# YifanXu74/MQ-Det

Hardware: AMD Instinct MI355X
Metric: images/sec MQ-GLIP-T 800×1333 5-shot vision queries, 1/2/4/8 MI355X (higher is better)
Workload: dtype f16; 1 GPU; BASELINE.json configs[1]: MQ-GLIP-T (Swin-T + BERT-base + GCP + 6-layer VLDyHead), 5 vision queries x 40 classes, 141-token caption, LVIS-style post-processing; every step a full forward (feature / language caches OFF; only host-side tokenizer / query-selection results are memoised)); global_batch=8, batch_per_gpu=8, image=800x1333 -> 800x1344, parallelism=dp1, weights=seeded random init (no checkpoints offline), residual_streams=fp32

## Files before the change

mq_det_amd/csrc/common.h:

```cpp
#pragma once
#include <hip/hip_runtime.h>
#include <stdint.h>

#if defined(MQ_F32)
typedef float half_t;
typedef float half8 __attribute__((ext_vector_type(8)));
typedef float half4 __attribute__((ext_vector_type(4)));
typedef float half2_ __attribute__((ext_vector_type(2)));
#define MQ_SYM(name) name##_f32
#define MQ_NAMESPACE_BEGIN namespace mq_f32 {
#define MQ_NAMESPACE_END }
#elif defined(MQ_BF16)
typedef __bf16 half_t;
typedef __bf16 half8 __attribute__((ext_vector_type(8)));
typedef __bf16 half4 __attribute__((ext_vector_type(4)));
typedef __bf16 half2_ __attribute__((ext_vector_type(2)));
#define MQ_SYM(name) name##_bf16
#define MQ_NAMESPACE_BEGIN namespace mq_bf16 {
#define MQ_NAMESPACE_END }
#else
typedef _Float16 half_t;
typedef _Float16 half8 __attribute__((ext_vector_type(8)));
typedef _Float16 half4 __attribute__((ext_vector_type(4)));
typedef _Float16 half2_ __attribute__((ext_vector_type(2)));
#define MQ_SYM(name) name
#define MQ_NAMESPACE_BEGIN
#define MQ_NAMESPACE_END
#endif
#if !defined(MQ_BF16) && !defined(MQ_F32)
#define MQ_PRIMARY_UNIT 1
#endif
#if defined(MQ_F32)
#define __expf(x) expf(x)
#define __builtin_amdgcn_exp2f(x) exp2f(x)
#define __builtin_amdgcn_rcpf(x) (1.0f / (x))
#endif
typedef float float4_ __attribute__((ext_vector_type(4)));
typedef float float2_ __attribute__((ext_vector_type(2)));

#define MQ_NEG_BIG (-1.0e30f)

#if defined(MQ_F32) && !defined(MQ_F32_EXACT)
typedef _Float16 mq_h16x8 __attribute__((ext_vector_type(8)));
struct mq_split8 { mq_h16x8 hi, lo; };
__device__ __forceinline__ mq_split8 mq_split(half8 x) {
  mq_split8 s;
#pragma unroll
  for (int i = 0; i < 8; ++i) {
    const _Float16 h = (_Float16)x[i];
    s.hi[i] = h;
    s.lo[i] = (_Float16)(__builtin_fmaf((float)h, -1.0f, x[i]) * 2048.0f);
  }
  return s;
}
__device__ __forceinline__ float4_ mfma16_split(const mq_split8& a, const mq_split8& b, float4_ c) {
#if defined(MQ_SIMT_EMULATION)
  return simt_mfma_16x16x32_split_frag(a.hi, a.lo, b.hi, b.lo, c);
#else
  float4_ t = {0.f, 0.f, 0.f, 0.f};
  c = __builtin_amdgcn_mfma_f32_16x16x32_f16(a.hi, b.hi, c, 0, 0, 0);
  t = __builtin_amdgcn_mfma_f32_16x16x32_f16(a.hi, b.lo, t, 0, 0, 0);
  t = __builtin_amdgcn_mfma_f32_16x16x32_f16(a.lo, b.hi, t, 0, 0, 0);
#pragma unroll
  for (int r = 0; r < 4; ++r) c[r] = __builtin_fmaf(t[r], 1.0f / 2048.0f, c[r]);
  return c;
#endif
}
typedef _Float16 mq_h16x4 __attribute__((ext_vector_type(4)));
typedef float mq_f32x4 __attribute__((ext_vector_type(4)));
__device__ __forceinline__ void mq_split4(mq_f32x4 x, mq_h16x4& hi, mq_h16x4& lo) {
#pragma unroll
  for (int i = 0; i < 4; ++i) {
    const _Float16 h = (_Float16)x[i];
    hi[i] = h;
    lo[i] = (_Float16)(__builtin_fmaf((float)h, -1.0f, x[i]) * 2048.0f);
  }
}
#endif

__device__ __forceinline__ float4_ mfma16(half8 a, half8 b, float4_ c) {
#if defined(MQ_F32) && !defined(MQ_F32_EXACT)
#if defined(MQ_SIMT_EMULATION)
  return simt_mfma_16x16x32_split(a, b, c);
#else
  return mfma16_split(mq_split(a), mq_split(b), c);
#endif
#elif defined(MQ_F32)
#if defined(MQ_SIMT_EMULATION)
  return simt_mfma_16x16x32_f32_8x4(a, b, c);
#else
#pragma unroll
  for (int j = 0; j < 8; ++j) c = __builtin_amdgcn_mfma_f32_16x16x4f32(a[j], b[j], c, 0, 0, 0);
  return c;
#endif
#elif defined(MQ_BF16)
  return __builtin_amdgcn_mfma_f32_16x16x32_bf16(a, b, c, 0, 0, 0);
#else
  return __builtin_amdgcn_mfma_f32_16x16x32_f16(a, b, c, 0, 0, 0);
#endif
}

__device__ __forceinline__ half8 zero8() {
  half8 z;
#pragma unroll
  for (int i = 0; i < 8; ++i) z[i] = (half_t)0.f;
  return z;
}

typedef __fp16 mq_fp16x4_t __attribute__((__vector_size__(8)));
__device__ __forceinline__ half4 lds_read_tr16(const half_t* p) {
#if defined(MQ_F32)
  const int l = __lane_id(), base = l & ~15, i = l & 15;
  half4 o;
#pragma unroll
  for (int j = 0; j < 4; ++j) {
    const half_t* src = (const half_t*)__shfl((unsigned long long)p, base + 4 * j + (i >> 2));
    o[j] = src[i & 3];
  }
  return o;
#else
  mq_fp16x4_t v = __builtin_amdgcn_ds_read_tr16_b64_v4f16((__attribute__((address_space(3))) mq_fp16x4_t*)p);
  half4 o;
  __builtin_memcpy(&o, &v, 8);
  return o;
#endif
}

typedef _Float16 mq_h16x4_t __attribute__((ext_vector_type(4)));
__device__ __forceinline__ mq_h16x4_t lds_read_tr16_h(const _Float16* p) {
  mq_fp16x4_t v = __builtin_amdgcn_ds_read_tr16_b64_v4f16((__attribute__((address_space(3))) mq_fp16x4_t*)p);
  mq_h16x4_t o;
  __builtin_memcpy(&o, &v, 8);
  return o;
}

__device__ __forceinline__ void lds_stage_frag8(const half_t* src_lane, half_t* dst_base, int lane) {
#if defined(MQ_F32)
  *(half8*)(dst_base + lane * 8) = *(const half8*)src_lane;
  asm volatile("s_waitcnt lgkmcnt(0)" ::: "memory");
#else
  (void)lane;
  __builtin_amdgcn_global_load_lds((const __attribute__((address_space(1))) void*)src_lane, (__attribute__((address_space(3))) void*)dst_base, 16, 0, 0);
#endif
}

typedef __amdgpu_buffer_rsrc_t mq_rsrc;
__device__ __forceinline__ mq_rsrc mq_raw_buffer(const void* base) { return __builtin_amdgcn_make_buffer_rsrc((void*)base, 0, 0x7fffffff, 0x00020000); }
__device__ __forceinline__ void lds_stage_frag8_buf(mq_rsrc r, const half_t* base, int eoff, int leoff, half_t* dst_base, int lane) {
#if defined(MQ_F32)
  (void)r;
  lds_stage_frag8(base + eoff + leoff, dst_base, lane);
#else
  (void)base; (void)lane;
  __builtin_amdgcn_raw_ptr_buffer_load_lds(r, (__attribute__((address_space(3))) void*)dst_base, 16, leoff * (int)sizeof(half_t), eoff * (int)sizeof(half_t), 0, 0);
#endif
}
__device__ __forceinline__ void lds_stage_16b_buf(mq_rsrc r, int boff, int lboff, void* dst_base) {
  __builtin_amdgcn_raw_ptr_buffer_load_lds(r, (__attribute__((address_space(3))) void*)dst_base, 16, lboff, boff, 0, 0);
}

__device__ __forceinline__ float group16_max(float v) {
  v = fmaxf(v, __shfl_xor(v, 1));
  v = fmaxf(v, __shfl_xor(v, 2));
  v = fmaxf(v, __shfl_xor(v, 4));
  v = fmaxf(v, __shfl_xor(v, 8));
  return v;
}
__device__ __forceinline__ float group16_sum(float v) {
  v += __shfl_xor(v, 1);
  v += __shfl_xor(v, 2);
  v += __shfl_xor(v, 4);
  v += __shfl_xor(v, 8);
  return v;
}
__device__ __forceinline__ float wave_sum(float v) {
#pragma unroll
  for (int o = 32; o > 0; o >>= 1) v += __shfl_xor(v, o);
  return v;
}
__device__ __forceinline__ float wave_max(float v) {
#pragma unroll
  for (int o = 32; o > 0; o >>= 1) v = fmaxf(v, __shfl_xor(v, o));
  return v;
}

__device__ __forceinline__ void wave_lds_fence() {
  asm volatile("s_waitcnt lgkmcnt(0)" ::: "memory");
  __builtin_amdgcn_wave_barrier();
}

static thread_local int mq_tl_dev = -1;
struct MqOncePerDevice {
  volatile bool set_[32] = {};
  bool first() {
    int dev = -1;
    if (hipGetDevice(&dev) != hipSuccess || dev < 0 || dev >= 32) { mq_tl_dev = -1; return true; }
    mq_tl_dev = dev;
    return !set_[dev];
  }
  void done() { if (mq_tl_dev >= 0) set_[mq_tl_dev] = true; }
};
struct MqMaxPerDevice {
  volatile size_t max_[32] = {};
  bool need(size_t bytes) {
    int dev = -1;
    if (hipGetDevice(&dev) != hipSuccess || dev < 0 || dev >= 32) { mq_tl_dev = -1; return true; }
    mq_tl_dev = dev;
    return bytes > max_[dev];
  }
  void done(size_t bytes) { if (mq_tl_dev >= 0 && bytes > max_[mq_tl_dev]) max_[mq_tl_dev] = bytes; }
};
static inline int mq_device_cus() {
  static int cus[32] = {};
  int dev = 0, n = 0;
  if (hipGetDevice(&dev) != hipSuccess || dev < 0 || dev >= 32) return 256;
  if (!cus[dev]) {
    if (hipDeviceGetAttribute(&n, hipDeviceAttributeMultiprocessorCount, dev) != hipSuccess || n <= 0) n = 256;
    cus[dev] = n;
  }
  return cus[dev];
}

#define MQ_CHECK_LAUNCH()                                   \
  do {                                                      \
    hipError_t e__ = hipGetLastError();                     \
    if (e__ != hipSuccess) return (int)e__;                 \
  } while (0)
```

mq_det_amd/csrc/vlfuse_attn.hip:

```cpp
#include "common.h"
#include <type_traits>
#include <cstdlib>

MQ_NAMESPACE_BEGIN

#if defined(MQ_F32) && !defined(MQ_F32_EXACT)
#define MQ_VL_SPLIT 1
typedef mq_split8 vfrag;
__device__ __forceinline__ vfrag vl_frag(half8 x) { return mq_split(x); }
__device__ __forceinline__ float4_ vl_mfma(const vfrag& a, const vfrag& b, float4_ c) { return mfma16_split(a, b, c); }
#else
#define MQ_VL_SPLIT 0
typedef half8 vfrag;
__device__ __forceinline__ vfrag vl_frag(half8 x) { return x; }
__device__ __forceinline__ float4_ vl_mfma(vfrag a, vfrag b, float4_ c) { return mfma16(a, b, c); }
#endif

namespace {
constexpr int VH = 8, VD = 256;
constexpr int BM = 128;
constexpr int TK = 64;
constexpr int KS = VD + 16;
constexpr int TILE = TK * KS;
using S0 = std::integral_constant<int, 0>;
using S1 = std::integral_constant<int, 1>;
}

struct I2TParams {
  const half_t* v;
  const half_t* kf;
  const half_t* vo;
  long kv_bs, kv_hs, kv_ts;
  const float* bias;
  const int* kv_len;
  const half_t* obias;
  half_t* out;
  int B, N, T;
  int H;
  float clamp;
};

template <int NTH> struct TileRegs { half8 r[2048 / NTH]; };

template <int I, int N, class F>
__device__ __forceinline__ void static_for_u_impl(F& f) {
  if constexpr (I < N) {
    f(std::integral_constant<int, I>{});
    static_for_u_impl<I + 1, N>(f);
  }
}
template <int N, class F>
__device__ __forceinline__ void static_for_u(F f) { static_for_u_impl<0, N>(f); }

template <int NTH, int NCH = 2048 / NTH>
__device__ __forceinline__ void tile_issue(TileRegs<NTH>& t, const half_t* src, int row0, int last_row, int tid, int ld = VD) {
#pragma unroll
  for (int i = 0; i < NCH; ++i) {
    const int c = tid + i * NTH;
    const int row = min(row0 + (c >> 5), last_row);
    t.r[i] = *(const half8*)(src + (row * ld + (c & 31) * 8));
  }
}
template <int NTH, int NCH = 2048 / NTH>
__device__ __forceinline__ void tile_commit(const TileRegs<NTH>& t, half_t* dst, int tid) {
#pragma unroll
  for (int i = 0; i < NCH; ++i) {
    const int c = tid + i * NTH;
#if MQ_VL_SPLIT
    const mq_split8 sp = mq_split(t.r[i]);
    _Float16* h = (_Float16*)dst + (c >> 5) * KS + (c & 31) * 8;
    *(mq_h16x8*)h = sp.hi;
    *(mq_h16x8*)(h + TILE) = sp.lo;
#else
    *(half8*)(dst + (c >> 5) * KS + (c & 31) * 8) = t.r[i];
#endif
  }
}

template <bool QLDS, int QB, int NBL = 4>
__device__ __forceinline__ void qk_tile(const half_t* tile, const vfrag (&qf)[QB][8], const half_t* qw, float4_ (&s)[4][QB],
                                        int l15, int lg) {
  static_assert(!(MQ_VL_SPLIT && QLDS), "split-precise: the Q fragments live in registers (a planar Q tile does not fit beside the key tiles)");
#pragma unroll
  for (int nb = 0; nb < 4; ++nb)
#pragma unroll
    for (int qb = 0; qb < QB; ++qb) s[nb][qb] = (float4_){0.f, 0.f, 0.f, 0.f};
#pragma unroll
  for (int kk = 0; kk < VD / 32; ++kk) {
    vfrag kf[4], qq[QB];
#pragma unroll
    for (int nb = 0; nb < NBL; ++nb) {
#if MQ_VL_SPLIT
      const _Float16* kp = (const _Float16*)tile + (nb * 16 + l15) * KS + kk * 32 + lg * 8;
      kf[nb].hi = *(const mq_h16x8*)kp;
      kf[nb].lo = *(const mq_h16x8*)(kp + TILE);
#else
      kf[nb] = *(const half8*)(tile + (nb * 16 + l15) * KS + kk * 32 + lg * 8);
#endif
    }
#pragma unroll
    for (int qb = 0; qb < QB; ++qb) {
#if !MQ_VL_SPLIT
      if constexpr (QLDS) qq[qb] = *(const half8*)(qw + (qb * 16 + l15) * KS + kk * 32 + lg * 8);
      else
#endif
      qq[qb] = qf[qb][kk];
    }
#pragma unroll
    for (int nb = 0; nb < NBL; ++nb)
#pragma unroll
      for (int qb = 0; qb < QB; ++qb) s[nb][qb] = vl_mfma(kf[nb], qq[qb], s[nb][qb]);
  }
}

template <int QB, int STL = 2>
__device__ __forceinline__ void pv_tile(const half_t* tile, const half8 (&pf)[2][QB], float4_ (&o)[16][QB], int l15, int lg) {
#pragma unroll
  for (int st = 0; st < STL; ++st) {
#if MQ_VL_SPLIT
    const _Float16* base = (const _Float16*)tile + (st * 32 + 4 * lg + (l15 >> 2)) * KS + (l15 & 3) * 4;
    vfrag pq[QB];
#pragma unroll
    for (int qb = 0; qb < QB; ++qb) pq[qb] = mq_split(pf[st][qb]);
#pragma unroll
    for (int db = 0; db < 16; ++db) {
      vfrag a;
      const mq_h16x4_t h0 = lds_read_tr16_h(base + db * 16), h1 = lds_read_tr16_h(base + 16 * KS + db * 16);
      const mq_h16x4_t l0 = lds_read_tr16_h(base + TILE + db * 16), l1 = lds_read_tr16_h(base + TILE + 16 * KS + db * 16);
#pragma unroll
      for (int j = 0; j < 4; ++j) { a.hi[j] = h0[j]; a.hi[4 + j] = h1[j]; a.lo[j] = l0[j]; a.lo[4 + j] = l1[j]; }
#pragma unroll
      for (int qb = 0; qb < QB; ++qb) o[db][qb] = vl_mfma(a, pq[qb], o[db][qb]);
    }
#else
    const half_t* base = tile + (st * 32 + 4 * lg + (l15 >> 2)) * KS + (l15 & 3) * 4;
#pragma unroll
    for (int db = 0; db < 16; ++db) {
      const half4 lo = lds_read_tr16(base + db * 16);
      const half4 hi = lds_read_tr16(base + 16 * KS + db * 16);
      half8 a;
#pragma unroll
      for (int j = 0; j < 4; ++j) { a[j] = lo[j]; a[4 + j] = hi[j]; }
#pragma unroll
      for (int qb = 0; qb < QB; ++qb) o[db][qb] = mfma16(a, pf[st][qb], o[db][qb]);
    }
#endif
  }
}

template <int NT, int QB, int NBL, int ABL = 0, bool QREG = false>
__global__ __launch_bounds__(2048 / (QB * 4)) void vlfuse_i2t_kernel(I2TParams p) {
  constexpr bool LEAN = NT >= 3 && !QREG && !MQ_VL_SPLIT;
  constexpr bool ONE = LEAN || MQ_VL_SPLIT;
  constexpr int NTH = 2048 / (QB * 4), WR = 16 * QB;
  extern __shared__ __attribute__((aligned(16))) char smem[];
  half_t* tiles = (half_t*)smem;
  half_t* Qs = tiles + 2 * TILE;
  float* bias_s = (float*)(Qs + (LEAN ? BM * KS : 0));

  const int tid = threadIdx.x, wave = tid >> 6, lane = tid & 63;
  const int l15 = lane & 15, lg = lane >> 4;
  const int qtiles = (p.N + BM - 1) / BM;
  const long total = (long)p.B * qtiles;
  const int per = (int)((total + 7) >> 3);
  const int wslot = blockIdx.x >> 3;
  const long w = (long)(blockIdx.x & 7) * per + wslot;
  if (wslot >= per || w >= total) return;
  const int b = (int)(w / qtiles);
  const int qtile = (int)(w - (long)b * qtiles);
  const int row0 = qtile * BM + wave * WR;

  float* mask_s = bias_s + VH * NT * TK;
  const int kv_eff = p.kv_len ? max(1, min(p.T, p.kv_len[b])) : p.T;
  for (int i = tid; i < p.H * NT * TK; i += NTH) {
    const int h = i / (NT * TK), t = i % (NT * TK);
    float v = MQ_NEG_BIG;
    if (t < kv_eff) v = p.bias ? p.bias[((long)b * p.H + h) * p.T + t] : 0.f;
    const bool masked = v < -1.0e29f;
    bias_s[i] = masked ? 0.f : v;
    mask_s[i] = masked ? MQ_NEG_BIG : 0.f;
  }
  const float cl2 = p.clamp > 0.f ? p.clamp : 3.0e38f;

  vfrag qf[QB][8];
  const half_t* vb = p.v + (long)b * p.N * VD;
  const half_t* qw = Qs + wave * WR * KS;
  if constexpr (LEAN) {
    TileRegs<NTH> q0, q1;
    tile_issue(q0, vb, qtile * BM, p.N - 1, tid);
    tile_issue(q1, vb, qtile * BM + 64, p.N - 1, tid);
    tile_commit(q0, Qs, tid);
    tile_commit(q1, Qs + 64 * KS, tid);
  } else {
#pragma unroll
    for (int qb = 0; qb < QB; ++qb) {
      const int row = min(row0 + qb * 16 + l15, p.N - 1);
#pragma unroll
      for (int kk = 0; kk < 8; ++kk) qf[qb][kk] = vl_frag(*(const half8*)(vb + (long)row * VD + kk * 32 + lg * 8));
    }
  }

  float4_ o[16][QB];
#pragma unroll
  for (int db = 0; db < 16; ++db)
#pragma unroll
    for (int qb = 0; qb < QB; ++qb) o[db][qb] = (float4_){0.f, 0.f, 0.f, 0.f};

  constexpr int PER_HEAD = 2 * NT;
  const int U = p.H * PER_HEAD;
  TileRegs<NTH> slot[ONE ? 1 : 2];
  if constexpr (ABL != 0) {
#pragma unroll
    for (int i = 0; i < 2048 / NTH; ++i) { slot[0].r[i] = zero8(); slot[ONE ? 0 : 1].r[i] = zero8(); }
  }
  auto rounds_of = [](int np) constexpr {
    if (np < 0) return 2048 / NTH;
    np %= 2 * NT;
    const int j = np % NT, rows = j != NT - 1 ? 64 : (np < NT ? 16 * NBL : 32 * ((NBL + 1) / 2));
    return (rows * 32 + NTH - 1) / NTH;
  };
  auto issue = [&](auto SLOT, auto NP, int u) {
    constexpr int sl = decltype(SLOT)::value, np = decltype(NP)::value;
    u = min(u, U - 1);
    const int h = u / PER_HEAD, j = u % PER_HEAD;
    const half_t* src = (j < NT ? p.kf : p.vo) + (long)b * p.kv_bs + (long)h * p.kv_hs;
    if constexpr (!(ABL & 1)) tile_issue<NTH, rounds_of(np)>(slot[sl], src, (j < NT ? j : j - NT) * TK, p.T - 1, tid, (int)p.kv_ts);
  };
  auto begin = [&](auto POS, int u) {
    constexpr int pos = decltype(POS)::value, par = pos & 1;
    if constexpr (ONE) issue(S0{}, std::integral_constant<int, pos + 1>{}, u + 1);
    else issue(std::integral_constant<int, par>{}, std::integral_constant<int, pos + 2>{}, u + 2);
    __builtin_amdgcn_sched_barrier(0);
  };
  auto end = [&](auto POS) {
    constexpr int pos = decltype(POS)::value, par = pos & 1;
    __builtin_amdgcn_sched_barrier(0);
    if constexpr (!(ABL & 2)) tile_commit<NTH, rounds_of((pos + 1) % PER_HEAD)>(slot[ONE ? 0 : (par ^ 1)], tiles + (par ^ 1) * TILE, tid);
    __syncthreads();
  };
  issue(S0{}, std::integral_constant<int, -1>{}, 0);
  if constexpr (!ONE) issue(S1{}, std::integral_constant<int, -1>{}, 1);
  tile_commit(slot[0], tiles, tid);
  __syncthreads();

  for (int h = 0; h < p.H; ++h) {
    const int u0 = h * PER_HEAD;
    float4_ s[NT][4][QB];
    auto qk_step = [&](auto J) {
      constexpr int j = decltype(J)::value;
      begin(J, u0 + j);
      if constexpr (!(ABL & 8)) qk_tile<LEAN, QB, (j == NT - 1 ? NBL : 4)>(tiles + (j & 1) * TILE, qf, qw, s[j], l15, lg);
      else {
#pragma unroll
        for (int nb = 0; nb < 4; ++nb)
#pragma unroll
          for (int qb = 0; qb < QB; ++qb) s[j][nb][qb] = (float4_){0.f, 0.f, 0.f, 0.f};
      }
#pragma unroll
      for (int nb = 0; nb < (j == NT - 1 ? NBL : 4); ++nb) {
        const float4_ kb = *(const float4_*)(bias_s + (h * NT + j) * TK + nb * 16 + 4 * lg);
        const float4_ km = *(const float4_*)(mask_s + (h * NT + j) * TK + nb * 16 + 4 * lg);
#pragma unroll
        for (int r = 0; r < 4; ++r)
#pragma unroll
          for (int qb = 0; qb < QB; ++qb)
            s[j][nb][qb][r] = __builtin_amdgcn_fmed3f(s[j][nb][qb][r] + kb[r], -cl2, cl2) + km[r];
      }
      end(J);
    };
    qk_step(std::integral_constant<int, 0>{});
    if constexpr (NT > 1) qk_step(std::integral_constant<int, 1>{});
    if constexpr (NT > 2) qk_step(std::integral_constant<int, 2>{});
    if constexpr (NT > 3) qk_step(std::integral_constant<int, 3>{});

#pragma unroll
    for (int qb = 0; qb < ((ABL & 4) ? 0 : QB); ++qb) {
      float mx = MQ_NEG_BIG;
#pragma unroll
      for (int j = 0; j < NT; ++j)
#pragma unroll
        for (int nb = 0; nb < (j == NT - 1 ? NBL : 4); ++nb)
#pragma unroll
          for (int r = 0; r < 4; ++r) mx = fmaxf(mx, s[j][nb][qb][r]);
      mx = fmaxf(mx, __shfl_xor(mx, 16));
      mx = fmaxf(mx, __shfl_xor(mx, 32));
      float sum = 0.f;
#pragma unroll
      for (int j = 0; j < NT; ++j)
#pragma unroll
        for (int nb = 0; nb < (j == NT - 1 ? NBL : 4); ++nb)
#pragma unroll
          for (int r = 0; r < 4; ++r) {
            const float e = __expf(s[j][nb][qb][r] - mx);
            s[j][nb][qb][r] = e;
            sum += e;
          }
      sum += __shfl_xor(sum, 16);
      sum += __shfl_xor(sum, 32);
      const float inv = __builtin_amdgcn_rcpf(sum);
#pragma unroll
      for (int j = 0; j < NT; ++j)
#pragma unroll
        for (int nb = 0; nb < (j == NT - 1 ? NBL : 4); ++nb)
#pragma unroll
          for (int r = 0; r < 4; ++r) s[j][nb][qb][r] *= inv;
    }
    auto pv_step = [&](auto J) {
      constexpr int j = decltype(J)::value;
      using POS = std::integral_constant<int, NT + j>;
      begin(POS{}, u0 + NT + j);
      half8 pf[2][QB];
#pragma unroll
      for (int st = 0; st < 2; ++st)
#pragma unroll
        for (int qb = 0; qb < QB; ++qb)
#pragma unroll
          for (int r = 0; r < 4; ++r) {
            constexpr int live = (j == NT - 1 ? NBL : 4);
            pf[st][qb][r] = 2 * st < live ? (half_t)s[j][2 * st][qb][r] : (half_t)0.f;
            pf[st][qb][4 + r] = 2 * st + 1 < live ? (half_t)s[j][2 * st + 1][qb][r] : (half_t)0.f;
          }
      if constexpr (!(ABL & 8)) pv_tile<QB, (j == NT - 1 ? (NBL + 1) / 2 : 2)>(tiles + ((NT + j) & 1) * TILE, pf, o, l15, lg);
      else {
#pragma unroll
        for (int qb = 0; qb < QB; ++qb)
#pragma unroll
          for (int r = 0; r < 4; ++r) o[0][qb][r] += (float)pf[0][qb][r] + (float)pf[1][qb][4 + r];
      }
      end(POS{});
    };
    pv_step(std::integral_constant<int, 0>{});
    if constexpr (NT > 1) pv_step(std::integral_constant<int, 1>{});
    if constexpr (NT > 2) pv_step(std::integral_constant<int, 2>{});
    if constexpr (NT > 3) pv_step(std::integral_constant<int, 3>{});
  }

  constexpr int OS = VD + 8;
  half_t* Os = tiles + wave * (WR * OS);
#pragma unroll
  for (int db = 0; db < 16; ++db)
#pragma unroll
    for (int qb = 0; qb < QB; ++qb) {
      half4 v4;
#pragma unroll
      for (int r = 0; r < 4; ++r) v4[r] = (half_t)o[db][qb][r];
      *(half4*)(Os + (qb * 16 + l15) * OS + db * 16 + 4 * lg) = v4;
    }
  wave_lds_fence();
  half_t* ob = p.out + (long)b * p.N * VD;
#pragma unroll
  for (int i = 0; i < 8 * QB; ++i) {
    const int c = lane + i * 64;
    const int rr = c >> 5, ch = c & 31;
    const int row = row0 + rr;
    if (row < p.N) {
      const half8 a = *(const half8*)(Os + rr * OS + ch * 8);
      const half8 res = *(const half8*)(vb + (long)row * VD + ch * 8);
      const half8 bb = *(const half8*)(p.obias + ch * 8);
      half8 y;
#pragma unroll
      for (int j = 0; j < 8; ++j) y[j] = (half_t)((float)a[j] + (float)res[j] + (float)bb[j]);
      *(half8*)(ob + (long)row * VD + ch * 8) = y;
    }
  }
}

template <int NT, int QB, int NBL, int ABL = 0, bool QREG = false>
static int launch_i2t(const I2TParams& p, hipStream_t stream) {
  constexpr size_t smem = (size_t)(2 * TILE + ((NT >= 3 && !QREG && !MQ_VL_SPLIT) ? BM * KS : 0)) * sizeof(half_t) + (size_t)2 * VH * NT * TK * sizeof(float);
  static_assert(4 * 32 * (VD + 8) <= 2 * TILE, "O staging must fit in the tiles");
  static MqOncePerDevice attr_set;
  if (attr_set.first()) {
    hipError_t e = hipFuncSetAttribute((const void*)vlfuse_i2t_kernel<NT, QB, NBL, ABL, QREG>, hipFuncAttributeMaxDynamicSharedMemorySize, (int)smem);
    if (e != hipSuccess) return (int)e;
    attr_set.done();
  }
  const int qtiles = (p.N + BM - 1) / BM;
  const long per = ((long)p.B * qtiles + 7) / 8;
  hipLaunchKernelGGL((vlfuse_i2t_kernel<NT, QB, NBL, ABL, QREG>), dim3((unsigned)(8 * per)), dim3(2048 / (QB * 4)), smem, stream, p);
  MQ_CHECK_LAUNCH();
  return 0;
}


static int vlfuse_qb() {
  static const int qb = [] { const char* e = getenv("MQ_VLFUSE_QB"); return (e && e[0] == '2') ? 2 : 1; }();
  return qb;
}

extern "C" int MQ_SYM(mq_vlfuse_i2t_fwd)(const void* v_ln, const void* kf, const void* vo, long kv_bs, long kv_hs, long kv_ts, const float* bias,
                                 const int* kv_len, const void* out_bias, void* out, int B, int N, int T, int heads, int max_kv, float clamp,
                                 int variant, void* stream) {
  if (B <= 0 || N <= 0) return 0;
  if (T < 1 || T > 256 || heads < 1 || heads > VH) return -1;
  if (kv_bs <= 0 && kv_hs <= 0 && kv_ts <= 0) { kv_ts = VD; kv_hs = (long)T * VD; kv_bs = (long)heads * T * VD; }
  constexpr long CH16 = 16 / (long)sizeof(half_t);
  if (kv_ts < VD || kv_ts * 256 >= (1l << 31) || (kv_bs | kv_hs | kv_ts) % CH16 || ((size_t)kf | (size_t)vo) % 16) return -6;
  I2TParams p;
  p.kv_bs = kv_bs; p.kv_hs = kv_hs; p.kv_ts = kv_ts;
  p.v = (const half_t*)v_ln; p.kf = (const half_t*)kf; p.vo = (const half_t*)vo; p.bias = bias; p.kv_len = kv_len;
  p.obias = (const half_t*)out_bias; p.out = (half_t*)out; p.B = B; p.N = N; p.T = T; p.H = heads; p.clamp = clamp;
  const int kv = (kv_len && max_kv > 0) ? min(max_kv, T) : T;
  const int nt = (kv + TK - 1) / TK;
  const int nbl = min(4, max(1, (kv - (nt - 1) * TK + 15) / 16));
  hipStream_t st = (hipStream_t)stream;
#ifdef MQ_PRIMARY_UNIT
  if (variant >= 100 && nt == 3 && nbl == 1) {
    switch (variant - 100) {
      case 1: return launch_i2t<3, 1, 1, 1>(p, st);
      case 3: return launch_i2t<3, 1, 1, 3>(p, st);
      case 4: return launch_i2t<3, 1, 1, 4>(p, st);
      case 8: return launch_i2t<3, 1, 1, 8>(p, st);
      case 11: return launch_i2t<3, 1, 1, 11>(p, st);
      case 15: return launch_i2t<3, 1, 1, 15>(p, st);
      default: return -4;
    }
  }
#endif
  if (variant != 1 && nt == 3 && nbl <= 2)
    return nbl == 1 ? launch_i2t<3, 1, 1, 0, true>(p, st) : launch_i2t<3, 1, 2, 0, true>(p, st);
#define MQ_I2T(NT_)                                                        \
  switch (nbl) {                                                           \
    case 1: return launch_i2t<NT_, 1, 1>(p, st);                           \
    case 2: return launch_i2t<NT_, 1, 2>(p, st);                           \
    case 3: return launch_i2t<NT_, 1, 3>(p, st);                           \
    default: return launch_i2t<NT_, 1, 4>(p, st);                          \
  }
  switch (nt) {
    case 1: MQ_I2T(1)
    case 2: MQ_I2T(2)
    case 3: MQ_I2T(3)
    default: MQ_I2T(4)
  }
#undef MQ_I2T
}

struct T2IParams {
  const half_t* kf;
  long kv_bs, kv_hs, kv_ts;
  const half_t* v;
  float* ws;
  half_t* out;
  const int* kv_len;
  const unsigned char* kmask;
  long kmask_bs;
  int H;
  int B, N, T, nsplit;
  int wr;
  int members;
  float clamp;
};
namespace { constexpr int WS_LD = VD + 4; }

template <class T, class F>
__device__ __forceinline__ void vl_scoped_tiles(T* __restrict__ b0, T* __restrict__ b1, F f) { f(b0, b1); }

template <int QB, bool KM, int ABL = 0, bool TDMA = false>
__global__ __launch_bounds__(2048 / (QB * 4)) void vlfuse_t2i_kernel(T2IParams p) {
  static_assert(!TDMA || (!MQ_VL_SPLIT && ABL == 0), "the LDS-copied tiles are the 16-bit builds' (the split-precise planes are computed while staging)");
  constexpr int NTH = 2048 / (QB * 4), WR = 16 * QB;
  extern __shared__ __attribute__((aligned(16))) char smem[];
  half_t* tiles = (half_t*)smem;

  const int tid = threadIdx.x, wave = tid >> 6, lane = tid & 63;
  const int l15 = lane & 15, lg = lane >> 4;
  const int members = p.members;
  const int seq = blockIdx.x >> 3;
  const int group = (seq / members) * 8 + (blockIdx.x & 7);
  if (group >= p.B * p.nsplit) return;
  const int wq = seq % members;
  const int b = group / p.nsplit, split = group % p.nsplit;
  const int kv_rows = p.kv_len ? max(1, min(p.T, p.kv_len[b])) : p.T;
  const int nblk = (kv_rows + WR - 1) / WR, units = p.H * nblk;
  if (wq * (NTH / 64) >= units) return;
  const int wv = __builtin_amdgcn_readfirstlane(wave);
  const int unit = wq * (NTH / 64) + wv;
  const bool wave_live = unit < units;
  const int h = wave_live ? unit / nblk : 0;
  const int row0 = (wave_live ? unit % nblk : 0) * WR;

  const int ntiles = (p.N + TK - 1) / TK;
  const int tps = (ntiles + p.nsplit - 1) / p.nsplit;
  const int t0 = split * tps, t1 = min(ntiles, t0 + tps);
  const int nt = max(t1 - t0, 0);

  vfrag qf[QB][8];
  const half_t* qb_ = p.kf + (long)b * p.kv_bs + (long)h * p.kv_hs;
#pragma unroll
  for (int qb = 0; qb < QB; ++qb) {
    const int row = min(row0 + qb * 16 + l15, p.T - 1);
#pragma unroll
    for (int kk = 0; kk < 8; ++kk) qf[qb][kk] = vl_frag(*(const half8*)(qb_ + (row * (int)p.kv_ts + kk * 32 + lg * 8)));
  }
  float4_ o[16][QB];
#pragma unroll
  for (int db = 0; db < 16; ++db)
#pragma unroll
    for (int qb = 0; qb < QB; ++qb) o[db][qb] = (float4_){0.f, 0.f, 0.f, 0.f};
  float m[QB], lsum[QB];
#pragma unroll
  for (int qb = 0; qb < QB; ++qb) { m[qb] = MQ_NEG_BIG; lsum[qb] = 0.f; }

  const half_t* vb = p.v + (long)b * p.N * VD;
  constexpr int RS = TDMA ? 0 : MQ_VL_SPLIT ? 1 : 2;
  TileRegs<NTH> slot[RS > 0 ? RS : 1];
  constexpr int NWV = NTH / 64, NPC = TK * KS * (int)sizeof(half_t) / 1024, PR = (NPC + NWV - 1) / NWV;
  static_assert(TK * KS * sizeof(half_t) % 1024 == 0, "a tile is a whole number of 1 KB pieces");
  int leoff[PR];
#pragma unroll
  for (int i = 0; i < PR; ++i) {
    const int gch = (wv + i * NWV) * 64 + lane, row = gch / (KS / 8), posn = gch % (KS / 8);
    leoff[i] = (row * VD + (posn < VD / 8 ? posn : 0) * 8) * (int)sizeof(half_t);
  }
  const mq_rsrc v_rsrc = __builtin_amdgcn_make_buffer_rsrc((void*)vb, 0, p.N * VD * (int)sizeof(half_t), 0x00020000);
  auto dma_tile = [&](int pos, half_t* buf) __attribute__((always_inline)) {
    const int t = t0 + min(pos, max(nt - 1, 0));
    const int toff = __builtin_amdgcn_readfirstlane(t * TK * VD * (int)sizeof(half_t));
#pragma unroll
    for (int i = 0; i < PR; ++i) {
      const int piece = wv + i * NWV;
      if (piece < NPC) lds_stage_16b_buf(v_rsrc, 0, toff + leoff[i], buf + piece * 512);
    }
  };
  if constexpr (ABL != 0) {
#pragma unroll
    for (int r = 0; r < RS; ++r)
#pragma unroll
      for (int i = 0; i < 2048 / NTH; ++i) slot[r].r[i] = zero8();
  }
  auto issue = [&](auto SLOT, int pos) {
    constexpr int sl = decltype(SLOT)::value;
    const int t = t0 + min(pos, max(nt - 1, 0));
    if constexpr (!(ABL & 1)) tile_issue(slot[sl], vb, t * TK, p.N - 1, tid);
  };
  const float cl = p.clamp > 0.f ? p.clamp : 3.0e38f;
  constexpr float THR = 8.0f;
  auto body = [&](auto PAR, auto SL, int pos, half_t* cur, half_t* nxt) __attribute__((always_inline)) {
    constexpr int sl = decltype(SL)::value;
    if constexpr (TDMA) dma_tile(pos + 1, nxt);
    else issue(SL, pos + RS);
    __builtin_amdgcn_sched_barrier(0);
    if (pos < nt && wave_live) {
      const half_t* tile = cur;
      float4_ s[4][QB];
      if constexpr (!(ABL & 8)) qk_tile<false, QB>(tile, qf, nullptr, s, l15, lg);
      else {
#pragma unroll
        for (int nb = 0; nb < 4; ++nb)
#pragma unroll
          for (int qb = 0; qb < QB; ++qb) s[nb][qb] = (float4_){0.f, 0.f, 0.f, 0.f};
      }
      const int key0 = (t0 + pos) * TK;
      unsigned km[4] = {0u, 0u, 0u, 0u};
      if constexpr (KM) {
#pragma unroll
        for (int nb = 0; nb < 4; ++nb) km[nb] = *(const unsigned*)(p.kmask + (long)b * p.kmask_bs + key0 + nb * 16 + 4 * lg);
      }
      float mx[QB];
#pragma unroll
      for (int qb = 0; qb < QB; ++qb) mx[qb] = MQ_NEG_BIG;
#pragma unroll
      for (int nb = 0; nb < 4; ++nb)
#pragma unroll
        for (int r = 0; r < 4; ++r) {
          const bool valid = key0 + nb * 16 + 4 * lg + r < p.N && (!KM || ((km[nb] >> (8 * r)) & 0xffu) == 0u);
#pragma unroll
          for (int qb = 0; qb < QB; ++qb) {
            float v = __builtin_amdgcn_fmed3f(s[nb][qb][r], -cl, cl);
            v = valid ? v : MQ_NEG_BIG;
            s[nb][qb][r] = v;
            mx[qb] = fmaxf(mx[qb], v);
          }
        }
      bool grow = false;
#pragma unroll
      for (int qb = 0; qb < QB; ++qb) {
        mx[qb] = fmaxf(mx[qb], __shfl_xor(mx[qb], 16));
        mx[qb] = fmaxf(mx[qb], __shfl_xor(mx[qb], 32));
        grow |= mx[qb] > m[qb] + THR;
      }
      if (__any(grow)) {
#pragma unroll
        for (int qb = 0; qb < QB; ++qb) {
          const float mnew = fmaxf(m[qb], mx[qb]);
          const float alpha = __expf(m[qb] - mnew);
          m[qb] = mnew;
          lsum[qb] *= alpha;
#pragma unroll
          for (int db = 0; db < 16; ++db)
#pragma unroll
            for (int r = 0; r < 4; ++r) o[db][qb][r] *= alpha;
        }
      }
      half8 pf[2][QB];
#pragma unroll
      for (int qb = 0; qb < QB; ++qb)
#pragma unroll
        for (int st = 0; st < 2; ++st)
#pragma unroll
          for (int r = 0; r < 4; ++r) {
            const float e0 = (ABL & 4) ? s[2 * st][qb][r] : __expf(s[2 * st][qb][r] - m[qb]);
            const float e1 = (ABL & 4) ? s[2 * st + 1][qb][r] : __expf(s[2 * st + 1][qb][r] - m[qb]);
            lsum[qb] += e0 + e1;
            pf[st][qb][r] = (half_t)e0;
            pf[st][qb][4 + r] = (half_t)e1;
          }
      if constexpr (!(ABL & 8)) pv_tile(tile, pf, o, l15, lg);
      else {
#pragma unroll
        for (int qb = 0; qb < QB; ++qb)
#pragma unroll
          for (int r = 0; r < 4; ++r) o[0][qb][r] += (float)pf[0][qb][r] + (float)pf[1][qb][4 + r];
      }
    }
    __builtin_amdgcn_sched_barrier(0);
    if constexpr (TDMA) __builtin_amdgcn_s_waitcnt(0x0F70);
    else if constexpr (!(ABL & 2)) tile_commit(slot[(sl + 1) % (RS > 0 ? RS : 1)], nxt, tid);
    __syncthreads();
  };
  if constexpr (TDMA) {
    dma_tile(0, tiles);
    __builtin_amdgcn_s_waitcnt(0x0F70);
    __syncthreads();
    vl_scoped_tiles(tiles, tiles + TILE, [&](half_t* b0, half_t* b1) __attribute__((always_inline)) {
      for (int pos = 0; pos < nt; pos += 2) {
        body(S0{}, S0{}, pos, b0, b1);
        if (pos + 1 < nt) body(S1{}, S0{}, pos + 1, b1, b0);
      }
    });
  } else {
  issue(S0{}, 0);
  if constexpr (RS >= 2) issue(S1{}, 1);
  if constexpr (RS == 3) issue(std::integral_constant<int, 2>{}, 2);
  tile_commit(slot[0], tiles, tid);
  __syncthreads();
  constexpr int U = RS == 3 ? 6 : 2;
  for (int pos = 0; pos < nt; pos += U) {
    bool done = false;
    static_for_u<U>([&](auto uc) __attribute__((always_inline)) {
      constexpr int u = decltype(uc)::value;
      if (!done) {
        body(std::integral_constant<int, u & 1>{}, std::integral_constant<int, u % (RS > 0 ? RS : 1)>{}, pos + u, tiles + (u & 1) * TILE, tiles + ((u & 1) ^ 1) * TILE);
        done = pos + u + 1 >= nt;
      }
    });
  }
  }

#pragma unroll
  for (int qb = 0; qb < QB; ++qb) {
    float l = lsum[qb];
    l += __shfl_xor(l, 16);
    l += __shfl_xor(l, 32);
    const int row = row0 + qb * 16 + l15;
    if (row < p.T && wave_live) {
      float* w = p.ws + (((long)split * p.B * p.H + (long)b * p.H + h) * p.T + row) * WS_LD;
#pragma unroll
      for (int db = 0; db < 16; ++db) *(float4_*)(w + db * 16 + 4 * lg) = o[db][qb];
      if (lg == 0) { w[VD] = m[qb]; w[VD + 1] = l; }
    }
  }
}

__global__ __launch_bounds__(256) void vlfuse_t2i_combine_kernel(T2IParams p) {
  const int lane = threadIdx.x & 63;
  const long gw = (long)blockIdx.x * 4 + (threadIdx.x >> 6);
  const long total = (long)p.B * p.H * p.T;
  if (gw >= total) return;
  const int row = gw % p.T;
  const int bh = gw / p.T, b = bh / p.H, h = bh % p.H;
  half_t* dst = p.out + ((long)b * p.T + row) * (p.H * VD) + h * VD + lane * 4;
  if (p.kv_len) {
    const int kv = max(1, min(p.T, p.kv_len[b]));
    if ((row / p.wr) * p.wr >= kv) {
      *(half4*)dst = (half4){(half_t)0.f, (half_t)0.f, (half_t)0.f, (half_t)0.f};
      return;
    }
  }
  const long stride = total * WS_LD;
  const float* base = p.ws + gw * WS_LD;
  float mx = MQ_NEG_BIG;
  for (int s = 0; s < p.nsplit; ++s) mx = fmaxf(mx, base[s * stride + VD]);
  float l = 0.f;
  float4_ acc = {0.f, 0.f, 0.f, 0.f};
  for (int s = 0; s < p.nsplit; ++s) {
    const float* w = base + s * stride;
    const float f = __expf(w[VD] - mx);
    l += w[VD + 1] * f;
    const float4_ v = *(const float4_*)(w + lane * 4);
    acc += v * f;
  }
  const float inv = 1.f / l;
  half4 y;
#pragma unroll
  for (int j = 0; j < 4; ++j) y[j] = (half_t)(acc[j] * inv);
  *(half4*)dst = y;
}

#ifdef MQ_PRIMARY_UNIT
extern "C" long mq_vlfuse_t2i_workspace_bytes(int B, int T, int nsplit) {
  return (long)(nsplit < 1 ? 1 : nsplit) * B * VH * T * WS_LD * (long)sizeof(float);
}
#endif

extern "C" int MQ_SYM(mq_vlfuse_t2i_fwd)(const void* kf, long kv_bs, long kv_hs, long kv_ts, const void* v_ln, const int* kv_len,
                                 const unsigned char* key_mask, long key_mask_bs,
                                 void* workspace, void* out, int B, int N, int T, int heads, int nsplit, int max_kv, float clamp,
                                 int variant, void* stream) {
  if (B <= 0 || T <= 0) return 0;
  if (N < 1 || workspace == nullptr || heads < 1 || heads > VH) return -1;
  if (kv_bs <= 0 && kv_hs <= 0 && kv_ts <= 0) { kv_ts = VD; kv_hs = (long)T * VD; kv_bs = (long)heads * T * VD; }
  if (kv_ts < VD || kv_ts * 256 >= (1l << 31) || (kv_bs | kv_hs | kv_ts) % (16 / (long)sizeof(half_t)) || (size_t)kf % 16) return -6;
  if (key_mask && ((key_mask_bs % 4) || key_mask_bs < (long)((N + TK - 1) / TK) * TK)) return -3;
  if (nsplit < 1) nsplit = 1;
  T2IParams p;
  p.kf = (const half_t*)kf; p.v = (const half_t*)v_ln; p.ws = (float*)workspace; p.out = (half_t*)out; p.kv_len = kv_len;
  p.kv_bs = kv_bs; p.kv_hs = kv_hs; p.kv_ts = kv_ts;
  p.B = B; p.N = N; p.T = T; p.H = heads; p.nsplit = nsplit; p.clamp = clamp; p.wr = 16 * vlfuse_qb();
  p.kmask = key_mask; p.kmask_bs = key_mask_bs;
  constexpr size_t smem = (size_t)2 * TILE * sizeof(half_t);
  static MqOncePerDevice attr_set;
  if (attr_set.first()) {
    hipError_t e = hipFuncSetAttribute((const void*)vlfuse_t2i_kernel<1, false>, hipFuncAttributeMaxDynamicSharedMemorySize, (int)smem);
    if (e == hipSuccess) e = hipFuncSetAttribute((const void*)vlfuse_t2i_kernel<2, false>, hipFuncAttributeMaxDynamicSharedMemorySize, (int)smem);
    if (e == hipSuccess) e = hipFuncSetAttribute((const void*)vlfuse_t2i_kernel<1, true>, hipFuncAttributeMaxDynamicSharedMemorySize, (int)smem);
    if (e == hipSuccess) e = hipFuncSetAttribute((const void*)vlfuse_t2i_kernel<2, true>, hipFuncAttributeMaxDynamicSharedMemorySize, (int)smem);
    if (e != hipSuccess) return (int)e;
    attr_set.done();
  }
  static const bool t2i_dma = [] { const char* e = getenv("MQ_VL_T2I_DMA"); return !(e && e[0] == '0'); }();
  (void)t2i_dma;
  const int rows = (kv_len && max_kv > 0) ? min(max_kv, T) : T;
  const int groups = B * nsplit, members = (heads * ((rows + p.wr - 1) / p.wr) + (128 / p.wr) - 1) / (128 / p.wr);
  p.members = members;
  const dim3 grid((unsigned)(8 * ((groups + 7) / 8) * members));
#ifdef MQ_PRIMARY_UNIT
  if (variant >= 100 && !key_mask) {
    hipStream_t st = (hipStream_t)stream;
    switch (variant - 100) {
#define MQ_T2I_ABL(A_)                                                                                                              \
      case A_: {                                                                                                                    \
        hipError_t e = hipFuncSetAttribute((const void*)vlfuse_t2i_kernel<1, false, A_>, hipFuncAttributeMaxDynamicSharedMemorySize, (int)smem); \
        if (e != hipSuccess) return (int)e;                                                                                         \
        hipLaunchKernelGGL((vlfuse_t2i_kernel<1, false, A_>), grid, dim3(512), smem, st, p);                                        \
        break;                                                                                                                      \
      }
      MQ_T2I_ABL(1) MQ_T2I_ABL(3) MQ_T2I_ABL(4) MQ_T2I_ABL(8) MQ_T2I_ABL(11) MQ_T2I_ABL(15)
#undef MQ_T2I_ABL
      default: return -4;
    }
    MQ_CHECK_LAUNCH();
    return 0;
  }
#endif
  if (vlfuse_qb() == 1) {
    if (key_mask) hipLaunchKernelGGL((vlfuse_t2i_kernel<1, true>), grid, dim3(512), smem, (hipStream_t)stream, p);
#if !MQ_VL_SPLIT
    else if (t2i_dma && (long)N * VD * (long)sizeof(half_t) < (1l << 31)) {
      static MqOncePerDevice attr_dma;
      if (attr_dma.first()) {
        hipError_t e = hipFuncSetAttribute((const void*)vlfuse_t2i_kernel<1, false, 0, true>, hipFuncAttributeMaxDynamicSharedMemorySize, (int)smem);
        if (e != hipSuccess) return (int)e;
        attr_dma.done();
      }
      hipLaunchKernelGGL((vlfuse_t2i_kernel<1, false, 0, true>), grid, dim3(512), smem, (hipStream_t)stream, p);
    }
#endif
    else hipLaunchKernelGGL((vlfuse_t2i_kernel<1, false>), grid, dim3(512), smem, (hipStream_t)stream, p);
  } else {
    if (key_mask) hipLaunchKernelGGL((vlfuse_t2i_kernel<2, true>), grid, dim3(256), smem, (hipStream_t)stream, p);
    else hipLaunchKernelGGL((vlfuse_t2i_kernel<2, false>), grid, dim3(256), smem, (hipStream_t)stream, p);
  }
  MQ_CHECK_LAUNCH();
  const long total = (long)B * heads * T;
  hipLaunchKernelGGL(vlfuse_t2i_combine_kernel, dim3((unsigned)((total + 3) / 4)), dim3(256), 0, (hipStream_t)stream, p);
  MQ_CHECK_LAUNCH();
  return 0;
}

MQ_NAMESPACE_END
```

Before: 516.7 images/sec.

## Fuse split-K combine into t2i attention kernel via last-arriver atomic ticket

Instead of launching a separate combine kernel after the split text-to-image attention, each wave increments a per-(batch, head, row-block) counter after writing its partial result. The last split to arrive merges all partials with the log-sum-exp rescale and writes the output. Rows beyond the covered blocks are zeroed inside the kernel. This removes one kernel launch and a full re-read pass, but adds a memset, atomics, threadfences and tail work on the last waves.

```diff
diff --git a/mq_det_amd/csrc/common.h b/mq_det_amd/csrc/common.h
--- a/mq_det_amd/csrc/common.h
+++ b/mq_det_amd/csrc/common.h
@@ -40,6 +40,11 @@
 
 #define MQ_NEG_BIG (-1.0e30f)
 
+#if defined(MQ_SIMT_EMULATION)
+inline void __threadfence() {}
+inline hipError_t hipMemsetAsync(void* p, int v, size_t n, hipStream_t) { memset(p, v, n); return hipSuccess; }
+#endif
+
 #if defined(MQ_F32) && !defined(MQ_F32_EXACT)
 typedef _Float16 mq_h16x8 __attribute__((ext_vector_type(8)));
 struct mq_split8 { mq_h16x8 hi, lo; };
diff --git a/mq_det_amd/csrc/vlfuse_attn.hip b/mq_det_amd/csrc/vlfuse_attn.hip
--- a/mq_det_amd/csrc/vlfuse_attn.hip
+++ b/mq_det_amd/csrc/vlfuse_attn.hip
@@ -449,8 +449,66 @@
   int wr;
   int members;
   float clamp;
+  int* cnt;
+  int nblk_t;
 };
 namespace { constexpr int WS_LD = VD + 4; }
+
+template <int WR>
+__device__ __forceinline__ void t2i_merge_unit(const T2IParams& p, int b, int h, int row0, int lane) {
+  constexpr int MS = 8;
+  const int l15 = lane & 15, lg = lane >> 4;
+  const int ns = p.nsplit;
+  const long stride = (long)p.B * p.H * p.T * WS_LD;
+  const float* unit = p.ws + ((long)b * p.H + h) * p.T * WS_LD;
+#pragma unroll 1
+  for (int r = 0; r < WR; r += 4) {
+    const int row = row0 + r + lg;
+    const float* base = unit + (long)min(row, p.T - 1) * WS_LD;
+    float2_ ml[MS];
+    float4_ v[MS][4];
+    auto fetch = [&](int s0) __attribute__((always_inline)) {
+#pragma unroll
+      for (int i = 0; i < MS; ++i) ml[i] = *(const float2_*)(base + min(s0 + i, ns - 1) * stride + VD);
+#pragma unroll
+      for (int i = 0; i < MS; ++i)
+#pragma unroll
+        for (int j = 0; j < 4; ++j) v[i][j] = *(const float4_*)(base + min(s0 + i, ns - 1) * stride + j * 64 + l15 * 4);
+    };
+    fetch(0);
+    float mx = MQ_NEG_BIG;
+#pragma unroll
+    for (int i = 0; i < MS; ++i)
+      if (i < ns) mx = fmaxf(mx, ml[i][0]);
+    for (int s = MS; s < ns; ++s) mx = fmaxf(mx, base[s * stride + VD]);
+    float l = 0.f;
+    float4_ acc[4];
+#pragma unroll
+    for (int j = 0; j < 4; ++j) acc[j] = (float4_){0.f, 0.f, 0.f, 0.f};
+    for (int s0 = 0; s0 < ns; s0 += MS) {
+      if (s0 > 0) fetch(s0);
+#pragma unroll
+      for (int i = 0; i < MS; ++i)
+        if (s0 + i < ns) {
+          const float f = __expf(ml[i][0] - mx);
+          l += ml[i][1] * f;
+#pragma unroll
+          for (int j = 0; j < 4; ++j) acc[j] += v[i][j] * f;
+        }
+    }
+    const float inv = 1.f / l;
+    if (row < p.T) {
+      half_t* dst = p.out + ((long)b * p.T + row) * (p.H * VD) + h * VD + l15 * 4;
+#pragma unroll
+      for (int j = 0; j < 4; ++j) {
+        half4 y;
+#pragma unroll
+        for (int k = 0; k < 4; ++k) y[k] = (half_t)(acc[j][k] * inv);
+        *(half4*)(dst + j * 64) = y;
+      }
+    }
+  }
+}
 
 template <class T, class F>
 __device__ __forceinline__ void vl_scoped_tiles(T* __restrict__ b0, T* __restrict__ b1, F f) { f(b0, b1); }
@@ -478,6 +536,12 @@
   const bool wave_live = unit < units;
   const int h = wave_live ? unit / nblk : 0;
   const int row0 = (wave_live ? unit % nblk : 0) * WR;
+  if (p.cnt && split == 0 && nblk * WR < p.T) {
+    const int nwg = min(members, (units + NTH / 64 - 1) / (NTH / 64));
+    const long n4 = (long)(p.T - nblk * WR) * p.H * (VD / 4);
+    half4* z = (half4*)(p.out + ((long)b * p.T + nblk * WR) * (p.H * VD));
+    for (long i = (long)wq * NTH + tid; i < n4; i += (long)nwg * NTH) z[i] = (half4){(half_t)0.f, (half_t)0.f, (half_t)0.f, (half_t)0.f};
+  }
 
   const int ntiles = (p.N + TK - 1) / TK;
   const int tps = (ntiles + p.nsplit - 1) / p.nsplit;
@@ -660,6 +724,15 @@
       if (lg == 0) { w[VD] = m[qb]; w[VD + 1] = l; }
     }
   }
+
+  if (p.cnt == nullptr || !wave_live) return;
+  __threadfence();
+  int ticket = 0;
+  if (lane == 0) ticket = atomicAdd(p.cnt + ((long)b * p.H + h) * p.nblk_t + row0 / WR, 1);
+  ticket = __builtin_amdgcn_readfirstlane(__shfl(ticket, 0));
+  if (ticket != p.nsplit - 1) return;
+  __threadfence();
+  t2i_merge_unit<WR>(p, b, h, row0, lane);
 }
 
 __global__ __launch_bounds__(256) void vlfuse_t2i_combine_kernel(T2IParams p) {
@@ -697,9 +770,11 @@
   *(half4*)dst = y;
 }
 
+static inline long t2i_partial_bytes(int B, int T, int nsplit) { return (long)(nsplit < 1 ? 1 : nsplit) * B * VH * T * WS_LD * (long)sizeof(float); }
+
 #ifdef MQ_PRIMARY_UNIT
 extern "C" long mq_vlfuse_t2i_workspace_bytes(int B, int T, int nsplit) {
-  return (long)(nsplit < 1 ? 1 : nsplit) * B * VH * T * WS_LD * (long)sizeof(float);
+  return t2i_partial_bytes(B, T, nsplit) + (long)B * VH * ((T + 15) / 16) * (long)sizeof(int);
 }
 #endif
 
@@ -718,6 +793,7 @@
   p.kv_bs = kv_bs; p.kv_hs = kv_hs; p.kv_ts = kv_ts;
   p.B = B; p.N = N; p.T = T; p.H = heads; p.nsplit = nsplit; p.clamp = clamp; p.wr = 16 * vlfuse_qb();
   p.kmask = key_mask; p.kmask_bs = key_mask_bs;
+  p.cnt = nullptr; p.nblk_t = (T + p.wr - 1) / p.wr;
   constexpr size_t smem = (size_t)2 * TILE * sizeof(half_t);
   static MqOncePerDevice attr_set;
   if (attr_set.first()) {
@@ -753,6 +829,12 @@
     return 0;
   }
 #endif
+  static const bool t2i_merge = [] { const char* e = getenv("MQ_VL_T2I_MERGE"); return !(e && e[0] == '0'); }();
+  if (t2i_merge) {
+    p.cnt = (int*)((char*)workspace + t2i_partial_bytes(B, T, nsplit));
+    hipError_t e = hipMemsetAsync(p.cnt, 0, (size_t)B * heads * p.nblk_t * sizeof(int), (hipStream_t)stream);
+    if (e != hipSuccess) return (int)e;
+  }
   if (vlfuse_qb() == 1) {
     if (key_mask) hipLaunchKernelGGL((vlfuse_t2i_kernel<1, true>), grid, dim3(512), smem, (hipStream_t)stream, p);
 #if !MQ_VL_SPLIT
@@ -772,6 +854,7 @@
     else hipLaunchKernelGGL((vlfuse_t2i_kernel<2, false>), grid, dim3(256), smem, (hipStream_t)stream, p);
   }
   MQ_CHECK_LAUNCH();
+  if (t2i_merge) return 0;
   const long total = (long)B * heads * T;
   hipLaunchKernelGGL(vlfuse_t2i_combine_kernel, dim3((unsigned)((total + 3) / 4)), dim3(256), 0, (hipStream_t)stream, p);
   MQ_CHECK_LAUNCH();
```

Result: slower. 489.1 images/sec (-5.3%).
